# zyhbili/Dual-Space-NeRF

Hardware: AMD Instinct MI355X
Metric: rendered rays/sec (64 samples/ray), 512x512 frame (higher is better)
Workload: dtype split-f16x3 (3 x v_mfma_f32_32x32x16_f16 on hi/lo fp16 operand halves, f32 accumulate: f32-equivalent accuracy - parity bars of the tests: 1e-4 absolute on RGB / acc / weights against the reference; sigma 1e-4 absolute where |sigma| <= 100 and 4e-6 RELATIVE to max|sigma| above (this checkpoint: |sig

## Files before the change

### dual-space-nerf_amd/csrc/dsn_nn.hip

```cpp
#include "dsn_common.h"
#include "dsn_kernels.h"
#include <cstdlib>

__global__ void __launch_bounds__(256) k_grid_params(const float4* __restrict__ cent, int F, float pad,
                                                      int target_cells, int maxcell, int cap, DsnGrid* __restrict__ g, int lazy) {
    __shared__ float s_lo[3][256], s_hi[3][256];
    const int t = threadIdx.x;
    float lo[3] = {INFINITY, INFINITY, INFINITY}, hi[3] = {-INFINITY, -INFINITY, -INFINITY};
    for (int f = t; f < F; f += 256) {
        const float4 c = cent[f];
        lo[0] = fminf(lo[0], c.x); lo[1] = fminf(lo[1], c.y); lo[2] = fminf(lo[2], c.z);
        hi[0] = fmaxf(hi[0], c.x); hi[1] = fmaxf(hi[1], c.y); hi[2] = fmaxf(hi[2], c.z);
    }
    for (int k = 0; k < 3; ++k) { s_lo[k][t] = lo[k]; s_hi[k][t] = hi[k]; }
    __syncthreads();
    for (int s = 128; s > 0; s >>= 1) {
        if (t < s)
            for (int k = 0; k < 3; ++k) {
                s_lo[k][t] = fminf(s_lo[k][t], s_lo[k][t + s]);
                s_hi[k][t] = fmaxf(s_hi[k][t], s_hi[k][t + s]);
            }
        __syncthreads();
    }
    if (t == 0) {
// ... 259 lines not shown
        constexpr int FILL_U = 4;
        while (todo) {
            int j[FILL_U];
            unsigned long long mk[FILL_U];
            float4 c[FILL_U];
#pragma unroll
            for (int u = 0; u < FILL_U; ++u) {
                j[u] = todo ? __ffsll((long long)todo) - 1 : -1;
                todo &= todo - 1;
                mk[u] = j[u] >= 0 ? __shfl(mine, j[u]) : 0ull;
                c[u] = make_float4(0.f, 0.f, 0.f, 0.f);
                if ((mk[u] >> lane) & 1ull) c[u] = cent[(j[u] << 6) + lane];
            }
#pragma unroll
            for (int u = 0; u < FILL_U; ++u) {
                if (j[u] < 0) continue;
                const int b0 = base + __shfl(front, j[u]);
                if ((mk[u] >> lane) & 1ull) {
                    const int at = b0 + __popcll(mk[u] & ((1ull << lane) - 1ull));
                    if (INLINE) reinterpret_cast<float4*>(list)[at] = c[u];
                    else reinterpret_cast<int32_t*>(list)[at] = __float_as_int(c[u].w);
                }
            }
        }
        return;
    }
    float blo[3], bhi[3];
    dsn_cell_box(g, cell, blo, bhi);
    const float m = u2[cell];
    constexpr int GRID_U = DSN_GRID_U;
    for (int f0 = 0; f0 < F; f0 += 64 * GRID_U) {
        float4 c[GRID_U];
#pragma unroll
        for (int u = 0; u < GRID_U; ++u) { const int f = f0 + 64 * u + lane; c[u] = cent[f < F ? f : 0]; }
#pragma unroll
        for (int u = 0; u < GRID_U; ++u) {
            const bool in = f0 + 64 * u + lane < F && dsn_in_list(dsn_box_dmin2(c[u], blo, bhi), m);
            const unsigned long long mask = __ballot(in);
            if (in) {
                const int at = base + __popcll(mask & ((1ull << lane) - 1ull));
                if (INLINE) reinterpret_cast<float4*>(list)[at] = c[u];
                else reinterpret_cast<int32_t*>(list)[at] = __float_as_int(c[u].w);
            }
            base += __popcll(mask);
        }
    }
}

static unsigned long long* dsn_member_words(const DsnGridView& vv) {
    const bool off = getenv("DSN_NN_NO_MEMBER") != nullptr;
    return (vv.super_cnt && !off) ? vv.member : nullptr;
}
static void dsn_build_level(const float4* cent, int F, const DsnGridView& v, float pad, int target, int maxcell, int cap,
                            bool inline_entries, hipStream_t st, bool params_only = false) {
    const int maxsuper = dsn_grid_maxsuper(maxcell);
    DsnGridView vv = v;
    if (getenv("DSN_NN_NO_SUPER")) vv.super_cnt = nullptr;
    hipLaunchKernelGGL(k_grid_params, dim3(1), dim3(256), 0, st, cent, F, pad, target, maxcell, cap, v.g, params_only ? 1 : 0);
    if (params_only) return;
    const int32_t* none = nullptr;
    if (vv.super_cnt)
        hipLaunchKernelGGL(k_grid_super, dim3(maxsuper), dim3(256), 0, st, cent, F, v.g, maxsuper, vv.super_cnt, vv.super_list, none, 0);
    hipLaunchKernelGGL(k_grid_count, dim3((maxcell + 3) / 4), dim3(256), 0, st, cent, F, v.g, v.u2, v.offsets, maxsuper,
                       (const int32_t*)vv.super_cnt, (const float4*)vv.super_list, none, 0, dsn_member_words(vv));
    dsn_launch_grid_scan(v, maxcell, 0, st);
    if (inline_entries)
        hipLaunchKernelGGL(k_grid_fill<true>, dim3((maxcell + 3) / 4), dim3(256), 0, st, cent, F, v.g, v.u2, v.offsets, v.list,
                           maxsuper, (const int32_t*)vv.super_cnt, (const float4*)vv.super_list, none, 0, (const unsigned long long*)dsn_member_words(vv));
    else
        hipLaunchKernelGGL(k_grid_fill<false>, dim3((maxcell + 3) / 4), dim3(256), 0, st, cent, F, v.g, v.u2, v.offsets, v.list,
                           maxsuper, (const int32_t*)vv.super_cnt, (const float4*)vv.super_list, none, 0, (const unsigned long long*)dsn_member_words(vv));
}

void dsn_launch_build_nn_visited(const float4* cent, int F, const DsnNNView& nn, const int32_t* visited, hipStream_t st) {
    const DsnGridView& v = nn.fine;
    const int maxcell = DSN_NN_FINE_MAXCELL, maxsuper = dsn_grid_maxsuper(maxcell);
    DsnGridView vv = v;
    if (getenv("DSN_NN_NO_SUPER")) vv.super_cnt = nullptr;
    if (getenv("DSN_LAZY_ALL_CELLS")) visited = nullptr;
    if (vv.super_cnt)
        hipLaunchKernelGGL(k_grid_super, dim3(maxsuper), dim3(256), 0, st, cent, F, v.g, maxsuper, vv.super_cnt, vv.super_list, visited, 1);
    hipLaunchKernelGGL(k_grid_count, dim3((maxcell + 3) / 4), dim3(256), 0, st, cent, F, v.g, v.u2, v.offsets, maxsuper,
                       (const int32_t*)vv.super_cnt, (const float4*)vv.super_list, visited, 1, dsn_member_words(vv));
    dsn_launch_grid_scan(v, maxcell, 1, st);
    hipLaunchKernelGGL(k_grid_fill<true>, dim3((maxcell + 3) / 4), dim3(256), 0, st, cent, F, v.g, v.u2, v.offsets, v.list,
                       maxsuper, (const int32_t*)vv.super_cnt, (const float4*)vv.super_list, visited, 1, (const unsigned long long*)dsn_member_words(vv));
}

__global__ void k_grid_complete(DsnGrid* __restrict__ g) {
    if (g->lazy == 3) { g->lazy = 0; g->ok = 1; }
}
void dsn_launch_build_nn_complete(const float4* cent, int F, const DsnNNView& nn, hipStream_t st) {
    const DsnGridView& v = nn.fine;
    const int maxcell = DSN_NN_FINE_MAXCELL, maxsuper = dsn_grid_maxsuper(maxcell);
    DsnGridView vv = v;
    if (getenv("DSN_NN_NO_SUPER")) vv.super_cnt = nullptr;
    const int32_t* none = nullptr;
    if (vv.super_cnt)
        hipLaunchKernelGGL(k_grid_super, dim3(maxsuper), dim3(256), 0, st, cent, F, v.g, maxsuper, vv.super_cnt, vv.super_list, none, 2);
    hipLaunchKernelGGL(k_grid_count, dim3((maxcell + 3) / 4), dim3(256), 0, st, cent, F, v.g, v.u2, v.offsets, maxsuper,
                       (const int32_t*)vv.super_cnt, (const float4*)vv.super_list, none, 2, dsn_member_words(vv));
    dsn_launch_grid_scan(v, maxcell, 2, st);
    hipLaunchKernelGGL(k_grid_fill<true>, dim3((maxcell + 3) / 4), dim3(256), 0, st, cent, F, v.g, v.u2, v.offsets, v.list,
                       maxsuper, (const int32_t*)vv.super_cnt, (const float4*)vv.super_list, none, 2, (const unsigned long long*)dsn_member_words(vv));
    hipLaunchKernelGGL(k_grid_complete, dim3(1), dim3(1), 0, st, v.g);
}

static int dsn_clampi(int x, int lo, int hi) { return x < lo ? lo : (x > hi ? hi : x); }

__global__ void k_grid_disable(DsnGrid* __restrict__ g) {
    g->ok = 0; g->ncell = 0; g->total = 0; g->nx = g->ny = g->nz = 0; g->lazy = 0;
    g->cap = 0; g->maxcell = 0;
}

void dsn_launch_build_nn(const float4* cent, int F, const DsnNNView& nn, float pad_fine, float pad_coarse, hipStream_t st,
                         bool fine_only, bool dense_fine, bool lazy) {
    int t_fine = dense_fine ? dsn_clampi(5 * F, 512, 62000) : dsn_clampi(3 * F, 512, 44000);
    if (!dense_fine) {
        static const long long tgt = [] { const char* e = getenv("DSN_NN_FINE_TARGET"); return e ? atoll(e) : 0ll; }();
        if (tgt > 0) t_fine = dsn_clampi((int)tgt, 512, 62000);
    }
    const int t_coarse = dsn_clampi(F / 3, 64, 5000);
    const char* ce = getenv("DSN_NN_FINE_CAP");
    const int fine_cap = ce && atoll(ce) > 0 && atoll(ce) < dsn_nn_fine_cap(F) ? (int)atoll(ce) : dsn_nn_fine_cap(F);
    dsn_build_level(cent, F, nn.fine, pad_fine, t_fine, DSN_NN_FINE_MAXCELL, fine_cap, true, st, lazy);
    if (fine_only || lazy) hipLaunchKernelGGL(k_grid_disable, dim3(1), dim3(1), 0, st, nn.coarse.g);
    else dsn_build_level(cent, F, nn.coarse, pad_coarse, t_coarse, DSN_NN_COARSE_MAXCELL, dsn_nn_coarse_cap(F), false, st);
}

#define NNS_THREADS 256
#ifndef NNS_SURVIVORS
#define NNS_SURVIVORS 320
#endif
#define NNS_PER 128

__device__ __forceinline__ void nns_point(const float* __restrict__ pts, const float* __restrict__ ray_o,
                                          const float* __restrict__ ray_d, const float* __restrict__ z_vals, int64_t i, int S,
                                          float* p) {
    if (pts) { p[0] = pts[3 * i]; p[1] = pts[3 * i + 1]; p[2] = pts[3 * i + 2]; return; }
    const int64_t ray = i / S;
    const float z = z_vals[i];
    p[0] = ray_o[3 * ray + 0] + ray_d[3 * ray + 0] * z;
    p[1] = ray_o[3 * ray + 1] + ray_d[3 * ray + 1] * z;
    p[2] = ray_o[3 * ray + 2] + ray_d[3 * ray + 2] * z;
}

__global__ void __launch_bounds__(NNS_THREADS) k_nns_classify(const DsnGrid* __restrict__ gf, const float* __restrict__ pts,
                                                              const float* __restrict__ ray_o, const float* __restrict__ ray_d,
                                                              const float* __restrict__ z_vals, int64_t N, int S,
                                                              int32_t* __restrict__ cell_of, int32_t* __restrict__ nn,
                                                              int32_t* __restrict__ counts, int32_t* __restrict__ outside) {
    const int64_t i = (int64_t)blockIdx.x * NNS_THREADS + threadIdx.x;
    if (gf->lazy) {
        if (i < N) { cell_of[i] = -1; if (nn) nn[i] = -1; }
        if (outside) {
            const unsigned long long om = __ballot(i < N);
            if (om && (threadIdx.x & 63) == 0) atomicAdd(outside, __popcll(om));
        }
        return;
    }
    float p[3] = {0.f, 0.f, 0.f};
    if (i < N) nns_point(pts, ray_o, ray_d, z_vals, i, S, p);
    const int c = dsn_nns_classify_one(gf, i, i < N, p[0], p[1], p[2], nullptr, cell_of, counts, outside);
    if (i < N && c < 0 && nn) nn[i] = -1;
}

__device__ __forceinline__ bool nns_lists_usable(const DsnGrid* __restrict__ gf, int lazy_call) { return gf->ok || (lazy_call && gf->lazy == 2); }
__global__ void __launch_bounds__(1024) k_nns_scan(const DsnGrid* __restrict__ gf, int32_t* __restrict__ counts,
                                                    int32_t* __restrict__ offs, int32_t* __restrict__ wave_offs,
                                                    int32_t* __restrict__ totals, int keep_counts, int lazy_call,
                                                    const int32_t* __restrict__ list_off = nullptr, int seg = 0) {
    __shared__ int s_n[1024 * SCAN_PER];
    __shared__ int s_w[16];
    const int ncell = nns_lists_usable(gf, lazy_call) ? gf->ncell : 0;
    auto waves_of = [&](int cell, int cnt) {
        int wv = (cnt + NNS_PER - 1) / NNS_PER;
        if (list_off && wv > 0 && cell < ncell) { const int len = list_off[cell + 1] - list_off[cell]; wv *= len > seg ? (len + seg - 1) / seg : 1; }
        return wv;
    };
    const int t = threadIdx.x;
    int carry_a = 0, carry_b = 0;
    for (int base = 0; base < ncell; base += 1024 * SCAN_PER) {
        for (int i = t; i < 1024 * SCAN_PER; i += 1024) s_n[i] = base + i < ncell ? counts[base + i] : 0;
        __syncthreads();
        int v[SCAN_PER], a = 0, b = 0;
#pragma unroll
        for (int k = 0; k < SCAN_PER; ++k) { v[k] = s_n[t * SCAN_PER + k]; a += v[k]; b += waves_of(base + t * SCAN_PER + k, v[k]); }
        int tot_a, tot_b;
        int ra = carry_a + dsn_block_exscan(a, s_w, tot_a);
        int rb = carry_b + dsn_block_exscan(b, s_w, tot_b);
#pragma unroll
        for (int k = 0; k < SCAN_PER; ++k) { s_n[t * SCAN_PER + k] = ra; ra += v[k]; }
        __syncthreads();
        for (int i = t; i < 1024 * SCAN_PER; i += 1024) if (base + i < ncell) offs[base + i] = s_n[i];
        __syncthreads();
#pragma unroll
        for (int k = 0; k < SCAN_PER; ++k) { s_n[t * SCAN_PER + k] = rb; rb += waves_of(base + t * SCAN_PER + k, v[k]); }
        __syncthreads();
        for (int i = t; i < 1024 * SCAN_PER; i += 1024)
            if (base + i < ncell) { wave_offs[base + i] = s_n[i]; if (!keep_counts) counts[base + i] = 0; }
        carry_a += tot_a; carry_b += tot_b;
        __syncthreads();
    }
    if (t == 0) { totals[0] = carry_b; totals[1] = carry_a; }
}

__global__ void __launch_bounds__(1024) k_nns_scan_mb(const DsnGrid* __restrict__ gf, const int32_t* __restrict__ counts,
                                                       int32_t* __restrict__ offs, int32_t* __restrict__ wave_offs,
                                                       int32_t* __restrict__ totals, int lazy_call,
                                                       const int32_t* __restrict__ list_off = nullptr, int seg = 0) {
    __shared__ int s_w[16];
    const int ncell = nns_lists_usable(gf, lazy_call) ? gf->ncell : 0;
    const int t = threadIdx.x, base = blockIdx.x * 1024;
    if (base >= ncell && blockIdx.x != 0) return;
    auto waves_of = [&](int cell, int cnt) {
        int wv = (cnt + NNS_PER - 1) / NNS_PER;
        if (list_off && wv > 0) { const int len = list_off[cell + 1] - list_off[cell]; wv *= len > seg ? (len + seg - 1) / seg : 1; }
        return wv;
    };
    int a = 0, b = 0;
    if (!list_off) {
        const int4* __restrict__ c4 = reinterpret_cast<const int4*>(counts);
        for (int i = t; i < base / 4; i += 1024) {
            const int4 c = c4[i];
            a += c.x + c.y + c.z + c.w;
            b += (c.x + NNS_PER - 1) / NNS_PER + (c.y + NNS_PER - 1) / NNS_PER + (c.z + NNS_PER - 1) / NNS_PER + (c.w + NNS_PER - 1) / NNS_PER;
        }
    } else {
        for (int i = t; i < base; i += 1024) { const int c = counts[i]; a += c; b += waves_of(i, c); }
    }
    int front_a, front_b, tot_a, tot_b;
    (void)dsn_block_exscan(a, s_w, front_a);
    (void)dsn_block_exscan(b, s_w, front_b);
    const int i = base + t;
    const int c = i < ncell ? counts[i] : 0, wv = i < ncell ? waves_of(i, c) : 0;
    const int ea = front_a + dsn_block_exscan(c, s_w, tot_a);
    const int eb = front_b + dsn_block_exscan(wv, s_w, tot_b);
    if (i < ncell) { offs[i] = ea; wave_offs[i] = eb; }
    if (t == 0 && base + 1024 >= ncell) { totals[0] = front_b + tot_b; totals[1] = front_a + tot_a; }
}
#define DSN_NN_SCAN_BLOCKS(maxcell) (((maxcell) + 1023) / 1024)

__global__ void __launch_bounds__(NNS_THREADS) k_nns_expand(const DsnGrid* __restrict__ gf, const int32_t* __restrict__ wave_offs,
                                                            const int32_t* __restrict__ totals, int32_t* __restrict__ wave_cell, int lazy_call) {
    const int c = blockIdx.x * NNS_THREADS + threadIdx.x;
    const int ncell = nns_lists_usable(gf, lazy_call) ? gf->ncell : 0;
    if (c >= ncell) return;
    const int w0 = wave_offs[c], w1 = (c + 1 < ncell) ? wave_offs[c + 1] : totals[0];
    for (int w = w0; w < w1; ++w) wave_cell[w] = c;
}

__global__ void __launch_bounds__(NNS_THREADS) k_nns_scatter(const int32_t* __restrict__ cell_of, const float* __restrict__ pts,
                                                             const float* __restrict__ ray_o, const float* __restrict__ ray_d,
                                                             const float* __restrict__ z_vals, int64_t N, int S,
                                                             const int32_t* __restrict__ offs, int32_t* __restrict__ cursor,
                                                             float4* __restrict__ sorted, const DsnGrid* __restrict__ gf = nullptr,
                                                             int32_t* __restrict__ cell_rw = nullptr, int32_t* __restrict__ outside = nullptr,
                                                             int lazy_call = 0) {
    const int64_t i = (int64_t)blockIdx.x * NNS_THREADS + threadIdx.x;
    const int lane = threadIdx.x & 63;
    if (gf && gf->lazy && !nns_lists_usable(gf, lazy_call)) {
        const bool mine = i < N && cell_rw[i] >= 0;
        if (mine) cell_rw[i] = -1;
        const unsigned long long m = __ballot(mine);
        if (m && lane == 0) atomicAdd(outside, __popcll(m));
        return;
    }
    const int c = i < N ? cell_of[i] : -1;
    const NnsRun r = nns_run(c, lane);
    int base = 0;
    if (r.head && c >= 0) base = offs[c] + atomicAdd(cursor + c, r.len);
    base = __shfl(base, r.head_lane);
    if (c >= 0) {
        float p[3];
        nns_point(pts, ray_o, ray_d, z_vals, i, S, p);
        sorted[base + r.rank] = make_float4(p[0], p[1], p[2], __int_as_float((int)i));
    }
}

__global__ void __launch_bounds__(NNS_THREADS) k_nns_scatter_ranked(int32_t* __restrict__ cell_of, const int32_t* __restrict__ rank_of,
                                                                    const float* __restrict__ ray_o, const float* __restrict__ ray_d,
                                                                    const float* __restrict__ z_vals, int64_t N, int S,
                                                                    const int32_t* __restrict__ offs, float4* __restrict__ sorted,
                                                                    const DsnGrid* __restrict__ gf, int32_t* __restrict__ outside, int lazy_call) {
    const int64_t i = (int64_t)blockIdx.x * NNS_THREADS + threadIdx.x;
    if (gf->lazy && !nns_lists_usable(gf, lazy_call)) {
        const bool mine = i < N && cell_of[i] >= 0;
        if (mine) cell_of[i] = -1;
        const unsigned long long m = __ballot(mine);
        if (m && (threadIdx.x & 63) == 0) atomicAdd(outside, __popcll(m));
        return;
    }
    if (i >= N) return;
    const int c = cell_of[i];
    if (c < 0) return;
    float p[3];
    nns_point(nullptr, ray_o, ray_d, z_vals, i, S, p);
    sorted[offs[c] + rank_of[i]] = make_float4(p[0], p[1], p[2], __int_as_float((int)i));
}

struct NnsWarp {
    const DsnFaceRec* face_world; const DsnFaceRec* face_canon; uint8_t* transparent; float* x_c; int32_t* active_list;
    int32_t* active_count; int lazy_canon;
};
template <bool WARP>
__global__ void __launch_bounds__(NNS_THREADS) k_nns_search(const int32_t* __restrict__ off_f, const float4* __restrict__ list_f,
                                                            const int32_t* __restrict__ wave_cell, const int32_t* __restrict__ wave_offs,
                                                            const int32_t* __restrict__ totals, const int32_t* __restrict__ offs,
                                                            const int32_t* __restrict__ counts, const float4* __restrict__ sorted,
                                                            int32_t* __restrict__ nn, NnsWarp wp, const float4* __restrict__ cent) {
    const int lane = threadIdx.x & 63;
    const unsigned bq = blockIdx.x >> 3, bx = blockIdx.x & 7u;
    const unsigned vb = ((bq >> 4) * 8u + bx) * 16u + (bq & 15u);
    const int w = __builtin_amdgcn_readfirstlane(vb * (NNS_THREADS / 64) + (threadIdx.x >> 6));
    const int nwaves = totals[0];
    if (WARP ? (int)(vb * (NNS_THREADS / 64)) >= nwaves : w >= nwaves) return;
    const bool wave_on = w < nwaves;
    const int c = __builtin_amdgcn_readfirstlane(wave_cell[wave_on ? w : 0]);
    const int slot = (w - __builtin_amdgcn_readfirstlane(wave_offs[c])) * NNS_PER + lane;
    const int cnt_c = __builtin_amdgcn_readfirstlane(counts[c]);
    const bool valid[2] = {wave_on && slot < cnt_c, wave_on && slot + 64 < cnt_c};
    float4 q[2] = {make_float4(0.f, 0.f, 0.f, 0.f), make_float4(0.f, 0.f, 0.f, 0.f)};
    const int so = __builtin_amdgcn_readfirstlane(offs[c]);
    if (valid[0]) q[0] = sorted[so + slot];
    if (valid[1]) q[1] = sorted[so + slot + 64];
    typedef float f32x2 __attribute__((ext_vector_type(2)));
    const f32x2 px = {q[0].x, q[1].x}, py = {q[0].y, q[1].y}, pz = {q[0].z, q[1].z};
    const int o = __builtin_amdgcn_readfirstlane(off_f[c]);
    const int n = wave_on ? __builtin_amdgcn_readfirstlane(off_f[c + 1]) - o : 0;
    const float4* __restrict__ e = list_f + o;
    float best[2] = {INFINITY, INFINITY};
    int bi[2] = {0, 0};
    auto step = [&](const float4 a) {
        const f32x2 cx = {a.x, a.x}, cy = {a.y, a.y}, cz = {a.z, a.z};
        const f32x2 dx = px - cx, dy = py - cy, dz = pz - cz;
        f32x2 d = dx * dx;
        d = __builtin_elementwise_fma(dy, dy, d);
        d = __builtin_elementwise_fma(dz, dz, d);
        const int id = __float_as_int(a.w);
        if (d.x < best[0]) { best[0] = d.x; bi[0] = id; }
        if (d.y < best[1]) { best[1] = d.y; bi[1] = id; }
    };
    int k = 0;
    if (!WARP && cent) {
        const int32_t* __restrict__ ids = reinterpret_cast<const int32_t*>(list_f) + o;
        auto at = [&](int f) { float4 a = cent[f]; a.w = __int_as_float(f); return a; };
        const bool single = cnt_c - (w - __builtin_amdgcn_readfirstlane(wave_offs[c])) * NNS_PER <= 64;
        if (single) {
            float b0 = INFINITY;
            int i0 = 0;
            const float qx = q[0].x, qy = q[0].y, qz = q[0].z;
            auto step1 = [&](const float4 a) {
                const float d = dsn_d2(qx, qy, qz, a);
                if (d < b0) { b0 = d; i0 = __float_as_int(a.w); }
            };
            constexpr int NB1 = 4;
            const int nb1 = n / NB1;
            int g1[NB1], g2[NB1];
            float4 c0[NB1], c1[NB1];
            if (nb1 > 0) {
#pragma unroll
                for (int j = 0; j < NB1; ++j) g1[j] = ids[j];
#pragma unroll
                for (int j = 0; j < NB1; ++j) c0[j] = at(g1[j]);
#pragma unroll
                for (int j = 0; j < NB1; ++j) g1[j] = ids[NB1 * (1 < nb1 ? 1 : 0) + j];
                for (int b = 0; b < nb1; ++b) {
                    if (b + 1 < nb1) {
#pragma unroll
                        for (int j = 0; j < NB1; ++j) c1[j] = at(g1[j]);
                    }
#pragma unroll
                    for (int j = 0; j < NB1; ++j) g2[j] = ids[NB1 * (b + 2 < nb1 ? b + 2 : 0) + j];
#pragma unroll
                    for (int j = 0; j < NB1; ++j) step1(c0[j]);
#pragma unroll
                    for (int j = 0; j < NB1; ++j) { c0[j] = c1[j]; g1[j] = g2[j]; }
                }
            }
            for (int kk = NB1 * nb1; kk < n; ++kk) step1(at(ids[kk]));
            if (valid[0]) nn[__float_as_int(q[0].w)] = i0;
            return;
        }
        constexpr int NB = 4;
        const int nb = n / NB;
        int f1[NB], f2[NB];
        float4 a0[NB], a1[NB];
        auto load_ids = [&](int b, int (&f)[NB]) {
#pragma unroll
            for (int j = 0; j < NB; ++j) f[j] = ids[NB * (b < nb ? b : 0) + j];
        };
        auto load_cent = [&](const int (&f)[NB], float4 (&a)[NB]) {
#pragma unroll
            for (int j = 0; j < NB; ++j) a[j] = at(f[j]);
        };
        if (nb > 0) {
            load_ids(0, f1);
            load_cent(f1, a0);
            load_ids(1, f1);
            for (int b = 0; b < nb; ++b) {
                if (b + 1 < nb) load_cent(f1, a1);
                load_ids(b + 2, f2);
#pragma unroll
                for (int j = 0; j < NB; ++j) step(a0[j]);
#pragma unroll
                for (int j = 0; j < NB; ++j) { a0[j] = a1[j]; f1[j] = f2[j]; }
            }
        }
        for (k = NB * nb; k < n; ++k) step(at(ids[k]));
    } else {
    bool pruned = false;
    int ns = 0;
#if !defined(DSN_NN_NO_PRUNE)
    __shared__ __attribute__((aligned(16))) float4 s_surv[NNS_THREADS / 64][NNS_SURVIVORS];
    float4* const surv = s_surv[threadIdx.x >> 6];
    if (n >= 96) {
        const float INF = INFINITY;
        float lo[3] = {fminf(valid[0] ? q[0].x : INF, valid[1] ? q[1].x : INF), fminf(valid[0] ? q[0].y : INF, valid[1] ? q[1].y : INF),
                       fminf(valid[0] ? q[0].z : INF, valid[1] ? q[1].z : INF)};
        float hi[3] = {fmaxf(valid[0] ? q[0].x : -INF, valid[1] ? q[1].x : -INF), fmaxf(valid[0] ? q[0].y : -INF, valid[1] ? q[1].y : -INF),
                       fmaxf(valid[0] ? q[0].z : -INF, valid[1] ? q[1].z : -INF)};
#pragma unroll
        for (int m = 32; m >= 1; m >>= 1)
#pragma unroll
            for (int a = 0; a < 3; ++a) {
                lo[a] = fminf(lo[a], __shfl_xor(lo[a], m));
                hi[a] = fmaxf(hi[a], __shfl_xor(hi[a], m));
            }
        float t = INF;
        for (int k0 = 0; k0 < n; k0 += 64) {
            if (k0 + lane < n) {
                const float4 a = e[k0 + lane];
                const float fx = fmaxf(fabsf(a.x - lo[0]), fabsf(a.x - hi[0])), fy = fmaxf(fabsf(a.y - lo[1]), fabsf(a.y - hi[1])),
                            fz = fmaxf(fabsf(a.z - lo[2]), fabsf(a.z - hi[2]));
                t = fminf(t, fx * fx + fy * fy + fz * fz);
            }
        }
#pragma unroll
        for (int m = 32; m >= 1; m >>= 1) t = fminf(t, __shfl_xor(t, m));
        t = t * 1.0001f;
        if (t < INF) {
            pruned = true;
            auto drain = [&]() {
                __builtin_amdgcn_wave_barrier();
                int j = 0;
                for (; j + 8 <= ns; j += 8) {
                    float4 a[8];
#pragma unroll
                    for (int u = 0; u < 8; ++u) a[u] = surv[j + u];
#pragma unroll
                    for (int u = 0; u < 8; ++u) step(a[u]);
                }
                for (; j < ns; ++j) step(surv[j]);
                __builtin_amdgcn_wave_barrier();
                ns = 0;
            };
            for (int k0 = 0; k0 < n; k0 += 64) {
                bool keep = false;
                float4 a = make_float4(0.f, 0.f, 0.f, 0.f);
                if (k0 + lane < n) {
                    a = e[k0 + lane];
                    const float gx = fmaxf(fmaxf(lo[0] - a.x, a.x - hi[0]), 0.0f), gy = fmaxf(fmaxf(lo[1] - a.y, a.y - hi[1]), 0.0f),
                                gz = fmaxf(fmaxf(lo[2] - a.z, a.z - hi[2]), 0.0f);
                    keep = !(gx * gx + gy * gy + gz * gz > t);
                }
                const unsigned long long mk = __ballot(keep);
                const int add = __popcll(mk);
                if (ns + add > NNS_SURVIVORS) drain();
                if (keep) surv[ns + __popcll(mk & ((1ull << lane) - 1ull))] = a;
                ns += add;
            }
            drain();
        }
    }
    if (!pruned) {
#endif
    for (; k + 8 <= n; k += 8) {
        float4 a[8];
#pragma unroll
        for (int j = 0; j < 8; ++j) a[j] = e[k + j];
#pragma unroll
        for (int j = 0; j < 8; ++j) step(a[j]);
    }
    for (; k < n; ++k) step(e[k]);
#if !defined(DSN_NN_NO_PRUNE)
    }
#endif
    }
    if (!WARP) {
        if (valid[0]) nn[__float_as_int(q[0].w)] = bi[0];
        if (valid[1]) nn[__float_as_int(q[1].w)] = bi[1];
        return;
    }
    bool active[2] = {false, false};
    int64_t idx[2];
#pragma unroll
    for (int h2 = 0; h2 < 2; ++h2) {
        idx[h2] = (int64_t)__float_as_int(q[h2].w);
        if (valid[h2]) {
            const float p[3] = {q[h2].x, q[h2].y, q[h2].z};
            const DsnFaceRec fw = dsn_load_face(wp.face_world, bi[h2]);
            float u, v, h, xc[3] = {0.f, 0.f, 0.f};
            dsn_project(p, fw, u, v, h);
            const bool tr = (u > 5.f) || (u < -4.f) || (v > 5.f) || (v < -4.f) || (fabsf(h) > 0.1f);
            if (!(tr && wp.lazy_canon)) {
                const DsnFaceRec fc = dsn_load_face(wp.face_canon, bi[h2]);
                dsn_map2face(u, v, h, fc, xc);
            }
            const int64_t i = idx[h2];
            wp.transparent[i] = tr ? 1 : 0;
            wp.x_c[3 * i] = xc[0]; wp.x_c[3 * i + 1] = xc[1]; wp.x_c[3 * i + 2] = xc[2];
            active[h2] = !tr;
        }
    }
    if (wp.active_list) {
        __shared__ int s_cnt[NNS_THREADS / 64][2];
        __shared__ int s_base;
        const unsigned long long m0 = __ballot(active[0]), m1 = __ballot(active[1]);
        const int wave = threadIdx.x >> 6;
        if (lane == 0) { s_cnt[wave][0] = __popcll(m0); s_cnt[wave][1] = __popcll(m1); }
        __syncthreads();
        if (threadIdx.x == 0) {
            int tot = 0;
            for (int kk = 0; kk < NNS_THREADS / 64; ++kk) tot += s_cnt[kk][0] + s_cnt[kk][1];
            s_base = tot ? atomicAdd(wp.active_count, tot) : 0;
        }
        __syncthreads();
        int off = s_base;
        for (int kk = 0; kk < wave; ++kk) off += s_cnt[kk][0] + s_cnt[kk][1];
        if (active[0]) wp.active_list[off + __popcll(m0 & ((1ull << lane) - 1ull))] = (int32_t)idx[0];
        if (active[1]) wp.active_list[off + s_cnt[wave][0] + __popcll(m1 & ((1ull << lane) - 1ull))] = (int32_t)idx[1];
    }
}

void dsn_launch_nn_cellmajor_warp(const DsnNNView& v, const float* ray_o, const float* ray_d, const float* z_vals, int64_t N, int S,
                                  int32_t* cell_of, void* sorted, void* small, const DsnFaceRec* face_world, const DsnFaceRec* face_canon,
                                  uint8_t* transparent, float* x_c, int32_t* active_list, int32_t* active_count, bool lazy_canon,
                                  int32_t** outside, hipStream_t st, bool classified, bool lazy_call) {
    char* q = (char*)small;
    int32_t* counts = (int32_t*)q;     q += dsn_align256(4 * (size_t)(DSN_NN_FINE_MAXCELL + 1));
    int32_t* offs = (int32_t*)q;       q += dsn_align256(4 * (size_t)(DSN_NN_FINE_MAXCELL + 1));
    int32_t* wave_offs = (int32_t*)q;  q += dsn_align256(4 * (size_t)(DSN_NN_FINE_MAXCELL + 1));
    int32_t* totals = (int32_t*)q;     q += 256;
    int32_t* wave_cell = (int32_t*)q;
    *outside = totals + 2;
    const dim3 gN((unsigned)((N + NNS_THREADS - 1) / NNS_THREADS)), b(NNS_THREADS);
    if (!classified) {
        (void)hipMemsetAsync(counts, 0, 4 * (size_t)(DSN_NN_FINE_MAXCELL + 1), st);
        (void)hipMemsetAsync(totals, 0, 256, st);
        hipLaunchKernelGGL(k_nns_classify, gN, b, 0, st, v.fine.g, (const float*)nullptr, ray_o, ray_d, z_vals, N, S, cell_of, (int32_t*)nullptr,
                           counts, totals + 2);
    }
    const bool ranked = classified && (lazy_call || !getenv("DSN_NN_ATOMIC_SCATTER"));
    const int lc = lazy_call ? 1 : 0;
    if (ranked)
        hipLaunchKernelGGL(k_nns_scan_mb, dim3(DSN_NN_SCAN_BLOCKS(DSN_NN_FINE_MAXCELL)), dim3(1024), 0, st, v.fine.g, (const int32_t*)counts, offs, wave_offs,
                           totals, lc, (const int32_t*)nullptr, 0);
    else
        hipLaunchKernelGGL(k_nns_scan, dim3(1), dim3(1024), 0, st, v.fine.g, counts, offs, wave_offs, totals, 0, lc);
    hipLaunchKernelGGL(k_nns_expand, dim3(DSN_NN_FINE_MAXCELL / NNS_THREADS), b, 0, st, v.fine.g, wave_offs, totals, wave_cell, lc);
    if (ranked)
        hipLaunchKernelGGL(k_nns_scatter_ranked, gN, b, 0, st, cell_of, (const int32_t*)(cell_of + N), ray_o, ray_d, z_vals, N, S, offs,
                           (float4*)sorted, (const DsnGrid*)v.fine.g, totals + 2, lc);
    else
        hipLaunchKernelGGL(k_nns_scatter, gN, b, 0, st, cell_of, (const float*)nullptr, ray_o, ray_d, z_vals, N, S, offs, counts, (float4*)sorted,
                           (const DsnGrid*)v.fine.g, cell_of, totals + 2, lc);
    const int64_t max_waves = N / NNS_PER + DSN_NN_FINE_MAXCELL + 1;
    const NnsWarp wp = {face_world, face_canon, transparent, x_c, active_list, active_count, lazy_canon ? 1 : 0};
    hipLaunchKernelGGL(k_nns_search<true>, dim3((unsigned)((max_waves + 3) / 4)), b, 0, st, v.fine.offsets, (const float4*)v.fine.list,
                       wave_cell, wave_offs, totals, offs, counts, (const float4*)sorted, (int32_t*)nullptr, wp, (const float4*)nullptr);
}

void dsn_nn_cellmajor_begin(void* small, int32_t** counts, int32_t** outside, hipStream_t st) {
    char* q = (char*)small;
    *counts = (int32_t*)q;
    int32_t* totals = (int32_t*)(q + 3 * dsn_align256(4 * (size_t)(DSN_NN_FINE_MAXCELL + 1)));
    *outside = totals + 2;
    (void)hipMemsetAsync(*counts, 0, 4 * (size_t)(DSN_NN_FINE_MAXCELL + 1), st);
    (void)hipMemsetAsync(totals, 0, 256, st);
}

size_t dsn_nn_sort_scratch_size(int64_t N) {
    return 3 * dsn_align256(4 * (size_t)(DSN_NN_FINE_MAXCELL + 1)) + 256 + dsn_align256(4 * (size_t)(N / 64 + DSN_NN_FINE_MAXCELL + 1));
}

void dsn_launch_nn_cellmajor(const DsnNNView& v, const float* pts, const float* ray_o, const float* ray_d, const float* z_vals,
                             int64_t N, int S, int32_t* cell_of, void* sorted, int32_t* nn, void* small, hipStream_t st) {
    char* q = (char*)small;
    int32_t* counts = (int32_t*)q;     q += dsn_align256(4 * (size_t)(DSN_NN_FINE_MAXCELL + 1));
    int32_t* offs = (int32_t*)q;       q += dsn_align256(4 * (size_t)(DSN_NN_FINE_MAXCELL + 1));
    int32_t* wave_offs = (int32_t*)q;  q += dsn_align256(4 * (size_t)(DSN_NN_FINE_MAXCELL + 1));
    int32_t* totals = (int32_t*)q;     q += 256;
    int32_t* wave_cell = (int32_t*)q;
    (void)hipMemsetAsync(counts, 0, 4 * (size_t)(DSN_NN_FINE_MAXCELL + 1), st);
    const dim3 gN((unsigned)((N + NNS_THREADS - 1) / NNS_THREADS)), b(NNS_THREADS);
    hipLaunchKernelGGL(k_nns_classify, gN, b, 0, st, v.fine.g, pts, ray_o, ray_d, z_vals, N, S, cell_of, nn, counts, (int32_t*)nullptr);
    hipLaunchKernelGGL(k_nns_scan, dim3(1), dim3(1024), 0, st, v.fine.g, counts, offs, wave_offs, totals, 0, 0);
    hipLaunchKernelGGL(k_nns_expand, dim3(DSN_NN_FINE_MAXCELL / NNS_THREADS), b, 0, st, v.fine.g, wave_offs, totals, wave_cell, 0);
    hipLaunchKernelGGL(k_nns_scatter, gN, b, 0, st, cell_of, pts, ray_o, ray_d, z_vals, N, S, offs, counts, (float4*)sorted);
    const int64_t max_waves = N / NNS_PER + DSN_NN_FINE_MAXCELL + 1;
    hipLaunchKernelGGL(k_nns_search<false>, dim3((unsigned)((max_waves + 3) / 4)), b, 0, st, v.fine.offsets, (const float4*)v.fine.list,
                       wave_cell, wave_offs, totals, offs, counts, (const float4*)sorted, nn, NnsWarp{}, (const float4*)nullptr);
}

__global__ void __launch_bounds__(NNS_THREADS) k_nns_classify_coarse(const DsnGrid* __restrict__ gf, const DsnGrid* __restrict__ gc,
                                                                     const float* __restrict__ pts, const uint8_t* __restrict__ live,
                                                                     int64_t N, int32_t* __restrict__ cell_of, int32_t* __restrict__ nn,
                                                                     int32_t* __restrict__ counts) {
    const int64_t i = (int64_t)blockIdx.x * NNS_THREADS + threadIdx.x;
    const int lane = threadIdx.x & 63;
    int c = -1;
    if (i < N && (!live || live[i])) {
        const float px = pts[3 * i], py = pts[3 * i + 1], pz = pts[3 * i + 2];
        if (dsn_grid_cell(*gf, px, py, pz) < 0) c = dsn_grid_cell(*gc, px, py, pz);
    }
    if (i < N) { cell_of[i] = c; if (c < 0) nn[i] = -1; }
    const NnsRun r = nns_run(c, lane);
    if (r.head && c >= 0) atomicAdd(counts + c, r.len);
}
#define NNS_FAR_SEG 768
__global__ void __launch_bounds__(NNS_THREADS) k_nns_search_far(const int32_t* __restrict__ off_c, const int32_t* __restrict__ list_c,
                                                                const int32_t* __restrict__ wave_cell, const int32_t* __restrict__ wave_offs,
                                                                const int32_t* __restrict__ totals, const int32_t* __restrict__ offs,
                                                                const int32_t* __restrict__ counts, const float4* __restrict__ sorted,
                                                                const float4* __restrict__ cent, unsigned long long* __restrict__ keys, int seg) {
    const int lane = threadIdx.x & 63;
    const int w = __builtin_amdgcn_readfirstlane(blockIdx.x * (NNS_THREADS / 64) + (threadIdx.x >> 6));
    if (w >= totals[0]) return;
    const int c = __builtin_amdgcn_readfirstlane(wave_cell[w]);
    const int cnt_c = __builtin_amdgcn_readfirstlane(counts[c]);
    const int chunks = (cnt_c + NNS_PER - 1) / NNS_PER;
    const int lw = w - __builtin_amdgcn_readfirstlane(wave_offs[c]);
    const int sg = lw / chunks, ch = lw - sg * chunks;
    const int slot = ch * NNS_PER + lane;
    const bool valid[2] = {slot < cnt_c, slot + 64 < cnt_c};
    float4 q[2] = {make_float4(0.f, 0.f, 0.f, 0.f), make_float4(0.f, 0.f, 0.f, 0.f)};
    const int so = __builtin_amdgcn_readfirstlane(offs[c]);
    if (valid[0]) q[0] = sorted[so + slot];
    if (valid[1]) q[1] = sorted[so + slot + 64];
    const int o = __builtin_amdgcn_readfirstlane(off_c[c]);
    const int len = __builtin_amdgcn_readfirstlane(off_c[c + 1]) - o;
    const int k0 = sg * seg;
    const int n = (len > seg ? (k0 + seg < len ? seg : len - k0) : len);
    const int32_t* __restrict__ ids = list_c + o + (len > seg ? k0 : 0);
    typedef float f32x2 __attribute__((ext_vector_type(2)));
    const f32x2 px = {q[0].x, q[1].x}, py = {q[0].y, q[1].y}, pz = {q[0].z, q[1].z};
    float best[2] = {INFINITY, INFINITY};
    int bi[2] = {0x7fffffff, 0x7fffffff};
    auto step = [&](const float4 a) {
        const f32x2 cx = {a.x, a.x}, cy = {a.y, a.y}, cz = {a.z, a.z};
        const f32x2 dx = px - cx, dy = py - cy, dz = pz - cz;
        f32x2 d = dx * dx;
        d = __builtin_elementwise_fma(dy, dy, d);
        d = __builtin_elementwise_fma(dz, dz, d);
        const int id = __float_as_int(a.w);
        if (d.x < best[0]) { best[0] = d.x; bi[0] = id; }
        if (d.y < best[1]) { best[1] = d.y; bi[1] = id; }
    };
    auto at = [&](int f) { float4 a = cent[f]; a.w = __int_as_float(f); return a; };
    constexpr int NB = 4;
    const int nb = n / NB;
    int f1[NB], f2[NB];
    float4 a0[NB], a1[NB];
    if (nb > 0) {
#pragma unroll
        for (int j = 0; j < NB; ++j) f1[j] = ids[j];
#pragma unroll
        for (int j = 0; j < NB; ++j) a0[j] = at(f1[j]);
#pragma unroll
        for (int j = 0; j < NB; ++j) f1[j] = ids[NB * (1 < nb ? 1 : 0) + j];
        for (int b = 0; b < nb; ++b) {
            if (b + 1 < nb) {
#pragma unroll
                for (int j = 0; j < NB; ++j) a1[j] = at(f1[j]);
            }
#pragma unroll
            for (int j = 0; j < NB; ++j) f2[j] = ids[NB * (b + 2 < nb ? b + 2 : 0) + j];
#pragma unroll
            for (int j = 0; j < NB; ++j) step(a0[j]);
#pragma unroll
            for (int j = 0; j < NB; ++j) { a0[j] = a1[j]; f1[j] = f2[j]; }
        }
    }
    for (int k = NB * nb; k < n; ++k) step(at(ids[k]));
#pragma unroll
    for (int h2 = 0; h2 < 2; ++h2)
        if (valid[h2] && best[h2] < INFINITY)
            atomicMin(keys + __float_as_int(q[h2].w), ((unsigned long long)__float_as_uint(best[h2]) << 32) | (unsigned)bi[h2]);
}
__global__ void __launch_bounds__(NNS_THREADS) k_nns_far_finish(const int32_t* __restrict__ cell_of, const unsigned long long* __restrict__ keys,
                                                                int64_t N, int32_t* __restrict__ nn) {
    const int64_t i = (int64_t)blockIdx.x * NNS_THREADS + threadIdx.x;
    if (i < N && cell_of[i] >= 0) nn[i] = (int32_t)(keys[i] & 0xffffffffull);
}
void dsn_launch_nn_cellmajor_coarse(const DsnNNView& v, const float4* cent, const float* pts, const uint8_t* live, int64_t N,
                                    int32_t* cell_of, void* sorted, int32_t* nn, void* small, hipStream_t st, void* keys8N, int F,
                                    int32_t* wave_scratch, int64_t wave_scratch_ints) {
    char* q = (char*)small;
    int32_t* counts = (int32_t*)q;     q += dsn_align256(4 * (size_t)(DSN_NN_FINE_MAXCELL + 1));
    int32_t* offs = (int32_t*)q;       q += dsn_align256(4 * (size_t)(DSN_NN_FINE_MAXCELL + 1));
    int32_t* wave_offs = (int32_t*)q;  q += dsn_align256(4 * (size_t)(DSN_NN_FINE_MAXCELL + 1));
    int32_t* totals = (int32_t*)q;     q += 256;
    int32_t* wave_cell = (int32_t*)q;
    static_assert(DSN_NN_COARSE_MAXCELL <= DSN_NN_FINE_MAXCELL, "the sort scratch is sized for the fine level");
    (void)hipMemsetAsync(counts, 0, 4 * (size_t)(DSN_NN_COARSE_MAXCELL + 1), st);
    const dim3 gN((unsigned)((N + NNS_THREADS - 1) / NNS_THREADS)), b(NNS_THREADS);
    hipLaunchKernelGGL(k_nns_classify_coarse, gN, b, 0, st, v.fine.g, v.coarse.g, pts, live, N, cell_of, nn, counts);
    static const bool seg_off = [] { const char* e = getenv("DSN_FAR_SEGMENTS"); return e && e[0] == '0'; }();
    static const int seg = [] { const char* e = getenv("DSN_FAR_SEG"); const int v = e ? atoi(e) : 0; return v >= 64 && v <= 16384 ? v & ~3 : NNS_FAR_SEG; }();
    const int64_t nseg_max = ((int64_t)F + seg - 1) / seg;
    const int64_t mw = (N / NNS_PER + DSN_NN_COARSE_MAXCELL + 1) * (nseg_max > 0 ? nseg_max : 1);
    if (keys8N && wave_scratch && !seg_off && mw + DSN_NN_COARSE_MAXCELL + 1 <= wave_scratch_ints) {
        wave_cell = wave_scratch;
        (void)hipMemsetAsync(keys8N, 0xff, 8 * (size_t)N, st);
        hipLaunchKernelGGL(k_nns_scan_mb, dim3(DSN_NN_SCAN_BLOCKS(DSN_NN_COARSE_MAXCELL)), dim3(1024), 0, st, v.coarse.g, (const int32_t*)counts, offs,
                           wave_offs, totals, 0, (const int32_t*)v.coarse.offsets, seg);
        hipLaunchKernelGGL(k_nns_expand, dim3(DSN_NN_COARSE_MAXCELL / NNS_THREADS), b, 0, st, v.coarse.g, wave_offs, totals, wave_cell, 0);
        int32_t* cursor = wave_cell + mw;
        (void)hipMemsetAsync(cursor, 0, 4 * (size_t)(DSN_NN_COARSE_MAXCELL + 1), st);
        hipLaunchKernelGGL(k_nns_scatter, gN, b, 0, st, cell_of, pts, (const float*)nullptr, (const float*)nullptr, (const float*)nullptr, N, 1,
                           offs, cursor, (float4*)sorted);
        hipLaunchKernelGGL(k_nns_search_far, dim3((unsigned)((mw + 3) / 4)), b, 0, st, v.coarse.offsets, (const int32_t*)v.coarse.list, wave_cell,
                           wave_offs, totals, offs, counts, (const float4*)sorted, cent, (unsigned long long*)keys8N, seg);
        hipLaunchKernelGGL(k_nns_far_finish, gN, b, 0, st, cell_of, (const unsigned long long*)keys8N, N, nn);
        return;
    }
    hipLaunchKernelGGL(k_nns_scan, dim3(1), dim3(1024), 0, st, v.coarse.g, counts, offs, wave_offs, totals, 0, 0);
    hipLaunchKernelGGL(k_nns_expand, dim3(DSN_NN_COARSE_MAXCELL / NNS_THREADS), b, 0, st, v.coarse.g, wave_offs, totals, wave_cell, 0);
    hipLaunchKernelGGL(k_nns_scatter, gN, b, 0, st, cell_of, pts, (const float*)nullptr, (const float*)nullptr, (const float*)nullptr, N, 1,
                       offs, counts, (float4*)sorted);
    const int64_t max_waves = N / NNS_PER + DSN_NN_COARSE_MAXCELL + 1;
    hipLaunchKernelGGL(k_nns_search<false>, dim3((unsigned)((max_waves + 3) / 4)), b, 0, st, v.coarse.offsets, (const float4*)v.coarse.list,
                       wave_cell, wave_offs, totals, offs, counts, (const float4*)sorted, nn, NnsWarp{}, cent);
}
```

Before: 29.00 million.

## Certify whole-wave transparency via bounding-box face tests to skip nearest-neighbor scans

```diff
diff --git a/dual-space-nerf_amd/csrc/dsn_nn.hip b/dual-space-nerf_amd/csrc/dsn_nn.hip
--- a/dual-space-nerf_amd/csrc/dsn_nn.hip
+++ b/dual-space-nerf_amd/csrc/dsn_nn.hip
@@ -585,9 +585,63 @@
 struct NnsWarp {
     const DsnFaceRec* face_world; const DsnFaceRec* face_canon; uint8_t* transparent; float* x_c; int32_t* active_list;
     int32_t* active_count; int lazy_canon;
+    int cert;
 };
+
+#define NNS_EPS 5.9604644775390625e-8f
+__device__ __forceinline__ bool nns_cert_face(const DsnFaceRec* __restrict__ recs, int fi, const float (&c)[3], const float (&r)[3]) {
+    const float4* fp = (const float4*)(recs + fi);
+    const float4 rm = fp[0], rn = fp[3];
+    const float m0[3] = {rm.x, rm.y, rm.z}, n[3] = {rn.x, rn.y, rn.z};
+    float t[3], Q = 0.f, S = 0.f, hc = 0.f, hr = 0.f;
+#pragma unroll
+    for (int k = 0; k < 3; ++k) {
+        t[k] = c[k] - m0[k];
+        const float T = fabsf(t[k]) + r[k];
+        Q += ((fabsf(c[k]) + r[k]) + fabsf(m0[k])) + T;
+        S += fabsf(n[k]) * T;
+        hc += n[k] * t[k];
+        hr += fabsf(n[k]) * r[k];
+    }
+    Q += 4.f * S;
+    const float mh = (128.f * NNS_EPS) * Q;
+    if (hc - hr > 0.1f + mh || hc + hr < -0.1f - mh) return true;
+    const float4 r10 = fp[1], r20 = fp[2];
+    const float v10[3] = {r10.x, r10.y, r10.z}, v20[3] = {r20.x, r20.y, r20.z};
+    const float d00 = rm.w, d01 = r10.w, d11 = r20.w, inv = rn.w;
+    const float n20 = (n[0] * v20[0] + n[1] * v20[1]) + n[2] * v20[2];
+    const float n10 = (n[0] * v10[0] + n[1] * v10[1]) + n[2] * v10[2];
+    float uc = 0.f, ur = 0.f, vc = 0.f, vr = 0.f, l20 = 0.f, l10 = 0.f;
+#pragma unroll
+    for (int k = 0; k < 3; ++k) {
+        const float p20 = v20[k] - n[k] * n20, p10 = v10[k] - n[k] * n10;
+        const float gu = inv * (d11 * p20 - d01 * p10), gv = inv * (d00 * p10 - d01 * p20);
+        uc += gu * t[k]; ur += fabsf(gu) * r[k];
+        vc += gv * t[k]; vr += fabsf(gv) * r[k];
+        l20 += fabsf(v20[k]); l10 += fabsf(v10[k]);
+    }
+    const float ai = (512.f * NNS_EPS) * Q * fabsf(inv);
+    const float mu = ai * (fabsf(d11) * l20 + fabsf(d01) * l10), mv = ai * (fabsf(d00) * l10 + fabsf(d01) * l20);
+    if (!(fabsf(inv) * (d00 * d11) < 1e4f)) return false;
+    return (mu < 1.f && (uc - ur > 5.f + mu || uc + ur < -4.f - mu)) || (mv < 1.f && (vc - vr > 5.f + mv || vc + vr < -4.f - mv));
+}
+#if defined(DSN_NN_CERT_STATS) && !defined(DSN_EXPERIMENTS)
+#error "DSN_NN_CERT_STATS is an experiment switch (debug counters): build with -DDSN_EXPERIMENTS"
+#endif
+#if defined(DSN_NN_CERT_STATS)
+__device__ unsigned long long g_nns_cert_stats[4];
+extern "C" __attribute__((visibility("default"))) int dsn_nn_cert_stats(unsigned long long* out4, int reset) {
+    if (hipDeviceSynchronize() != hipSuccess) return 1;
+    if (hipMemcpyFromSymbol(out4, HIP_SYMBOL(g_nns_cert_stats), sizeof(g_nns_cert_stats)) != hipSuccess) return 1;
+    if (reset) {
+        const unsigned long long z[4] = {0, 0, 0, 0};
+        if (hipMemcpyToSymbol(HIP_SYMBOL(g_nns_cert_stats), z, sizeof(z)) != hipSuccess) return 1;
+    }
+    return 0;
+}
+#endif
 template <bool WARP>
-__global__ void __launch_bounds__(NNS_THREADS) k_nns_search(const int32_t* __restrict__ off_f, const float4* __restrict__ list_f,
+__global__ void __launch_bounds__(NNS_THREADS) __attribute__((amdgpu_waves_per_eu(6))) k_nns_search(const int32_t* __restrict__ off_f, const float4* __restrict__ list_f,
                                                             const int32_t* __restrict__ wave_cell, const int32_t* __restrict__ wave_offs,
                                                             const int32_t* __restrict__ totals, const int32_t* __restrict__ offs,
                                                             const int32_t* __restrict__ counts, const float4* __restrict__ sorted,
@@ -624,6 +678,8 @@
         if (d.x < best[0]) { best[0] = d.x; bi[0] = id; }
         if (d.y < best[1]) { best[1] = d.y; bi[1] = id; }
     };
+    bool cert = WARP && wp.cert && n > 0;
+    float bc[3], br[3];
     int k = 0;
     if (!WARP && cent) {
         const int32_t* __restrict__ ids = reinterpret_cast<const int32_t*>(list_f) + o;
@@ -694,23 +750,45 @@
     } else {
     bool pruned = false;
     int ns = 0;
+    const float INF = INFINITY;
+    float lo[3] = {INF, INF, INF}, hi[3] = {-INF, -INF, -INF};
+    if (cert || n >= 96) {
+        lo[0] = fminf(valid[0] ? q[0].x : INF, valid[1] ? q[1].x : INF); lo[1] = fminf(valid[0] ? q[0].y : INF, valid[1] ? q[1].y : INF);
+        lo[2] = fminf(valid[0] ? q[0].z : INF, valid[1] ? q[1].z : INF);
+        hi[0] = fmaxf(valid[0] ? q[0].x : -INF, valid[1] ? q[1].x : -INF); hi[1] = fmaxf(valid[0] ? q[0].y : -INF, valid[1] ? q[1].y : -INF);
+        hi[2] = fmaxf(valid[0] ? q[0].z : -INF, valid[1] ? q[1].z : -INF);
+#pragma unroll
+        for (int m = 32; m >= 1; m >>= 1)
+#pragma unroll
+            for (int a = 0; a < 3; ++a) {
+                lo[a] = fminf(lo[a], __shfl_xor(lo[a], m));
+                hi[a] = fmaxf(hi[a], __shfl_xor(hi[a], m));
+            }
+#pragma unroll
+        for (int a = 0; a < 3; ++a) {
+            lo[a] = __int_as_float(__builtin_amdgcn_readfirstlane(__float_as_int(lo[a])));
+            hi[a] = __int_as_float(__builtin_amdgcn_readfirstlane(__float_as_int(hi[a])));
+        }
+    }
+    if (cert) {
+        const bool bad = (valid[0] && !(isfinite(q[0].x) && isfinite(q[0].y) && isfinite(q[0].z))) ||
+                         (valid[1] && !(isfinite(q[1].x) && isfinite(q[1].y) && isfinite(q[1].z)));
+        bool fin = true;
+#pragma unroll
+        for (int a = 0; a < 3; ++a) {
+            fin = fin && isfinite(lo[a]) && isfinite(hi[a]);
+            bc[a] = 0.5f * (lo[a] + hi[a]);
+            br[a] = fmaxf(hi[a] - bc[a], bc[a] - lo[a]) * (1.0f + 0x1p-20f);
+            bc[a] = __int_as_float(__builtin_amdgcn_readfirstlane(__float_as_int(bc[a])));
+            br[a] = __int_as_float(__builtin_amdgcn_readfirstlane(__float_as_int(br[a])));
+        }
+        cert = fin && __ballot(bad) == 0ull;
+    }
+    float t = INF;
 #if !defined(DSN_NN_NO_PRUNE)
     __shared__ __attribute__((aligned(16))) float4 s_surv[NNS_THREADS / 64][NNS_SURVIVORS];
     float4* const surv = s_surv[threadIdx.x >> 6];
     if (n >= 96) {
-        const float INF = INFINITY;
-        float lo[3] = {fminf(valid[0] ? q[0].x : INF, valid[1] ? q[1].x : INF), fminf(valid[0] ? q[0].y : INF, valid[1] ? q[1].y : INF),
-                       fminf(valid[0] ? q[0].z : INF, valid[1] ? q[1].z : INF)};
-        float hi[3] = {fmaxf(valid[0] ? q[0].x : -INF, valid[1] ? q[1].x : -INF), fmaxf(valid[0] ? q[0].y : -INF, valid[1] ? q[1].y : -INF),
-                       fmaxf(valid[0] ? q[0].z : -INF, valid[1] ? q[1].z : -INF)};
-#pragma unroll
-        for (int m = 32; m >= 1; m >>= 1)
-#pragma unroll
-            for (int a = 0; a < 3; ++a) {
-                lo[a] = fminf(lo[a], __shfl_xor(lo[a], m));
-                hi[a] = fmaxf(hi[a], __shfl_xor(hi[a], m));
-            }
-        float t = INF;
         for (int k0 = 0; k0 < n; k0 += 64) {
             if (k0 + lane < n) {
                 const float4 a = e[k0 + lane];
@@ -722,22 +800,36 @@
 #pragma unroll
         for (int m = 32; m >= 1; m >>= 1) t = fminf(t, __shfl_xor(t, m));
         t = t * 1.0001f;
-        if (t < INF) {
-            pruned = true;
-            auto drain = [&]() {
-                __builtin_amdgcn_wave_barrier();
-                int j = 0;
-                for (; j + 8 <= ns; j += 8) {
-                    float4 a[8];
-#pragma unroll
-                    for (int u = 0; u < 8; ++u) a[u] = surv[j + u];
-#pragma unroll
-                    for (int u = 0; u < 8; ++u) step(a[u]);
-                }
-                for (; j < ns; ++j) step(surv[j]);
-                __builtin_amdgcn_wave_barrier();
-                ns = 0;
-            };
+    }
+#endif
+    for (int k0 = 0; cert && k0 < n; k0 += 64) {
+        bool ok = true;
+        if (k0 + lane < n) {
+            const float4 a = e[k0 + lane];
+            const float gx = fmaxf(fmaxf(lo[0] - a.x, a.x - hi[0]), 0.0f), gy = fmaxf(fmaxf(lo[1] - a.y, a.y - hi[1]), 0.0f),
+                        gz = fmaxf(fmaxf(lo[2] - a.z, a.z - hi[2]), 0.0f);
+            if (!(gx * gx + gy * gy + gz * gz > t)) ok = nns_cert_face(wp.face_world, __float_as_int(a.w), bc, br);
+        }
+        cert = __ballot(!ok) == 0ull;
+    }
+#if !defined(DSN_NN_NO_PRUNE)
+    if (t < INF) {
+        pruned = true;
+        auto drain = [&]() {
+            __builtin_amdgcn_wave_barrier();
+            int j = 0;
+            for (; j + 8 <= ns; j += 8) {
+                float4 a[8];
+#pragma unroll
+                for (int u = 0; u < 8; ++u) a[u] = surv[j + u];
+#pragma unroll
+                for (int u = 0; u < 8; ++u) step(a[u]);
+            }
+            for (; j < ns; ++j) step(surv[j]);
+            __builtin_amdgcn_wave_barrier();
+            ns = 0;
+        };
+        if (!cert) {
             for (int k0 = 0; k0 < n; k0 += 64) {
                 bool keep = false;
                 float4 a = make_float4(0.f, 0.f, 0.f, 0.f);
@@ -756,8 +848,11 @@
             drain();
         }
     }
-    if (!pruned) {
+    const bool scan = !pruned && !cert;
+#else
+    const bool scan = !cert;
 #endif
+    if (scan) {
     for (; k + 8 <= n; k += 8) {
         float4 a[8];
 #pragma unroll
@@ -766,15 +861,20 @@
         for (int j = 0; j < 8; ++j) step(a[j]);
     }
     for (; k < n; ++k) step(e[k]);
-#if !defined(DSN_NN_NO_PRUNE)
-    }
-#endif
+    }
     }
     if (!WARP) {
         if (valid[0]) nn[__float_as_int(q[0].w)] = bi[0];
         if (valid[1]) nn[__float_as_int(q[1].w)] = bi[1];
         return;
     }
+#if defined(DSN_NN_CERT_STATS)
+    const unsigned long long ns2 = (unsigned long long)(__popcll(__ballot(valid[0])) + __popcll(__ballot(valid[1])));
+    if (WARP && wp.lazy_canon && wave_on && lane == 0) {
+        atomicAdd(&g_nns_cert_stats[0], 1ull); atomicAdd(&g_nns_cert_stats[2], ns2);
+        if (cert) { atomicAdd(&g_nns_cert_stats[1], 1ull); atomicAdd(&g_nns_cert_stats[3], ns2); }
+    }
+#endif
     bool active[2] = {false, false};
     int64_t idx[2];
 #pragma unroll
@@ -782,13 +882,16 @@
         idx[h2] = (int64_t)__float_as_int(q[h2].w);
         if (valid[h2]) {
             const float p[3] = {q[h2].x, q[h2].y, q[h2].z};
-            const DsnFaceRec fw = dsn_load_face(wp.face_world, bi[h2]);
             float u, v, h, xc[3] = {0.f, 0.f, 0.f};
-            dsn_project(p, fw, u, v, h);
-            const bool tr = (u > 5.f) || (u < -4.f) || (v > 5.f) || (v < -4.f) || (fabsf(h) > 0.1f);
-            if (!(tr && wp.lazy_canon)) {
-                const DsnFaceRec fc = dsn_load_face(wp.face_canon, bi[h2]);
-                dsn_map2face(u, v, h, fc, xc);
+            bool tr = true;
+            if (!cert) {
+                const DsnFaceRec fw = dsn_load_face(wp.face_world, bi[h2]);
+                dsn_project(p, fw, u, v, h);
+                tr = (u > 5.f) || (u < -4.f) || (v > 5.f) || (v < -4.f) || (fabsf(h) > 0.1f);
+                if (!(tr && wp.lazy_canon)) {
+                    const DsnFaceRec fc = dsn_load_face(wp.face_canon, bi[h2]);
+                    dsn_map2face(u, v, h, fc, xc);
+                }
             }
             const int64_t i = idx[h2];
             wp.transparent[i] = tr ? 1 : 0;
@@ -849,7 +952,9 @@
         hipLaunchKernelGGL(k_nns_scatter, gN, b, 0, st, cell_of, (const float*)nullptr, ray_o, ray_d, z_vals, N, S, offs, counts, (float4*)sorted,
                            (const DsnGrid*)v.fine.g, cell_of, totals + 2, lc);
     const int64_t max_waves = N / NNS_PER + DSN_NN_FINE_MAXCELL + 1;
-    const NnsWarp wp = {face_world, face_canon, transparent, x_c, active_list, active_count, lazy_canon ? 1 : 0};
+    const char* ce = getenv("DSN_NN_CERT");
+    const int cert = lazy_canon && !(ce && atoi(ce) == 0) ? 1 : 0;
+    const NnsWarp wp = {face_world, face_canon, transparent, x_c, active_list, active_count, lazy_canon ? 1 : 0, cert};
     hipLaunchKernelGGL(k_nns_search<true>, dim3((unsigned)((max_waves + 3) / 4)), b, 0, st, v.fine.offsets, (const float4*)v.fine.list,
                        wave_cell, wave_offs, totals, offs, counts, (const float4*)sorted, (int32_t*)nullptr, wp, (const float4*)nullptr);
 }
```

Result: no change. 29.15 million, median of 6 (+0.5%).
